# daisy9542/yolo-puncture

Hardware: AMD Instinct MI355X
Metric: images/sec (higher is better)
Workload: dtype bf16

## Files before the change

### include/yolop.h

```cpp
#ifndef YOLOP_H
#define YOLOP_H

#include <stddef.h>
#include <stdint.h>

#ifdef __cplusplus
extern "C" {
#endif

#define YP_OK 0
#define YP_ERR_ARG -1
#define YP_ERR_STATE -2
#define YP_ERR_HIP -3
#define YP_ERR_WEIGHT -4

#define YP_BF16 0
#define YP_F32 1

#define YP_TASK_DETECT 0
#define YP_TASK_SEGMENT 1

#define YP_NM 32
#define YP_MAX_MASKS 480
#define YP_MAX_DET 512
// ... 123 lines not shown
int yp_set_nms(yp_engine* e, float conf, float iou);

int yp_set_attention_form(yp_engine* e, int form);

int yp_set_autotune(yp_engine* e, int enable);

int yp_tuning_export(const yp_engine* e, int32_t* cfg_out, int cap);
int yp_tuning_import(yp_engine* e, int B, int H, int W, const int32_t* cfg, int n);

int yp_debug_force_conv_cfg(int cfg);
int yp_debug_op_cfg(const yp_engine* e, int i, int* cfg);
int yp_debug_last_store_form(void);
int yp_debug_max_workgroups(int n);
int yp_debug_conv_families(int* base, int* num_cfgs, int cap);
int yp_debug_ablation(int v);
int yp_debug_head_clocks(uint64_t* out8);
int yp_debug_attention(const void* qkv_dev, void* o_dev, int dtype, int B, int N, int nh, int kd, int hd, int q_stride, int q_coff, int o_stride,
                       int o_coff, int wgs, int* kernel_out, void* stream);
int yp_debug_attention_form(const void* qkv_dev, void* o_dev, int dtype, int B, int N, int nh, int kd, int hd, int q_stride, int q_coff, int o_stride,
                            int o_coff, int wgs, int form, int* kernel_out, void* stream);
int yp_debug_conv_s2(const void* x_dev, const void* w_dev, const float* bias_dev, const void* res_dev, void* y_dev, int out_f32, int B, int H,
                     int W, int Cin, int Cout, int silu, int cfg, int lds_weights, int64_t* lds_out, char* kernel_out, int kernel_cap,
                     void* stream);
int yp_debug_topk_anchors(const uint32_t* const mk_dev[3], int B, const int hw[3][2], int k, int32_t* sel_out_dev, uint32_t* thr_out_dev, void* stream);
int yp_debug_head_branch_clocks(uint64_t* out8);
int yp_debug_head_winners(yp_engine* e, int32_t* sel_host, float* box_host, float* coeff_host);
int yp_debug_contour_clocks(uint64_t* out12);
int yp_debug_pwsp_clocks(uint64_t* out32);

int yp_tuning_source(const yp_engine* e);

int yp_debug_host_selftest(yp_engine* e);
int yp_debug_graph_info(const yp_engine* e, int64_t* out6);
int yp_debug_head_positions(yp_engine* e, int64_t* out6);
int yp_debug_marker(void* stream);

int yp_set_graph(yp_engine* e, int enable);

#ifdef __cplusplus
}
#endif
#endif
```

### yolo-puncture_amd/csrc/common.h

```cpp
#pragma once
#include <hip/hip_runtime.h>
#include <stdint.h>
#include <atomic>
#include <cstdlib>
#include <string>
#include <vector>

namespace yp {

enum DType { DT_BF16 = 0, DT_F32 = 1 };
enum Act { ACT_NONE = 0, ACT_SILU = 1, ACT_RELU = 2 };

enum OpKind {
    OP_STEM = 0,
    OP_CONV = 1,
    OP_DWCONV = 2,
    OP_POOL5 = 3,
    OP_UPSAMPLE = 4,
    OP_ATTN = 5,
    OP_HEAD = 6,
    OP_CONVT = 7,
    OP_AMAX = 9,
    OP_POOL3 = 8,
};
// ... 253 lines not shown
void conv_dma_force_cfg(int cfg);
int conv_dma_forced_cfg();
void conv_set_debug_ablation(int v);
int conv_debug_ablation();
bool tile_balance_enabled(int family);

struct ConvFamily {
    int base, num_cfgs;
    bool (*valid)(const ConvParams& p, int c);
    std::string (*symbol)(const ConvParams& p, int c);
    hipError_t (*launch)(const ConvParams& p, int c, hipStream_t st);
    bool two_source;
    const char* tune_env;
    bool opt_in;
};
inline const char* res_f32_args(const ConvParams& p) { return p.out_f32 ? ",false,true" : p.res ? ",true,false" : ",false,false"; }
extern const ConvFamily conv_dma_family, conv_halo_family, conv_halo_p_family, conv_dma_p_family, conv_dma_lc_family, conv_halo_s2_family,
    conv_tile1_family, conv_wreg_family, conv_pxd_family, conv_ks_family, conv_wres_family, conv_wrs_family;
constexpr int kNumConvFamilies = 12;
extern const ConvFamily* const kConvFamilies[kNumConvFamilies];
int conv_halo_s2_pw_cfg(const ConvParams& p);
size_t conv_halo_s2_lds_bytes(const ConvParams& p, int c);
int conv_halo_s2_lds_weights(int on);
hipError_t launch_dwconv(const DwParams& p, int dtype, hipStream_t st);
std::string dwconv_kernel_name(const DwParams& p, int dtype);
hipError_t launch_stem(const StemParams& p, int dtype, hipStream_t st);
std::string stem_kernel_name(const StemParams& p, int dtype);
hipError_t launch_pool5(const PoolParams& p, int dtype, hipStream_t st);
hipError_t launch_sppf_pool3(const PoolParams& p, int dtype, hipStream_t st);
bool sppf_pool3_fits(const PoolParams& p, int dtype);
bool dwconv_mfma_valid(const DwParams& p, int dtype);
hipError_t launch_dwconv_mfma(const DwParams& p, hipStream_t st);
const char* dwconv_mfma_kernel_name(const DwParams& p);
hipError_t launch_upsample(const UpParams& p, int dtype, hipStream_t st);
enum AttnForm { ATTN_FORM_AUTO = 0, ATTN_FORM_STREAM = 1, ATTN_FORM_STREAM_WIDE = 3 };
inline bool attn_form_valid(int form) { return form == ATTN_FORM_AUTO || form == ATTN_FORM_STREAM || form == ATTN_FORM_STREAM_WIDE; }
constexpr int ATTN_RESIDENT_TOKENS = 400;
hipError_t launch_attention(const AttnParams& p, int dtype, hipStream_t st, int wgs = 0, int* kernel_out = nullptr, int form = ATTN_FORM_AUTO);
bool attention_fits(const AttnParams& p, int dtype, int* max_tokens, int form = ATTN_FORM_AUTO);
bool attention_takes_stream(const AttnParams& p, int dtype, int form);
bool attention_takes_stream_wide(const AttnParams& p, int dtype, int form);
bool attention_stream_scope(const AttnParams& p, int dtype);
void attention_stream_split(int B, int N, int nh, int wgs, int* nsplit_out, int* gpw_out);
hipError_t launch_attention_stream(const AttnParams& p, hipStream_t st, int wgs);
bool attention_stream_wide_scope(const AttnParams& p, int dtype);
hipError_t launch_attention_stream_wide(const AttnParams& p, hipStream_t st, int wgs);
// ... 118 lines not shown
```

### yolo-puncture_amd/csrc/conv_wres.hip

```cpp
#include "common.h"

namespace yp {

constexpr int WR_NW = 8;
constexpr int WR_MAXNF = 8;

template <int N, int FM, int NFW> __device__ __forceinline__ void wr_wait_lgkm(bf16x8 (&xs)[FM], bf16x8 (&ws)[NFW]) {
    static_assert(N >= 0 && N < 16, "lgkmcnt range");
    asm volatile("s_waitcnt lgkmcnt(%0)" : : "n"(N) : "memory");
#pragma unroll
    for (int f = 0; f < FM; ++f) asm volatile("" : "+v"(xs[f]));
#pragma unroll
    for (int i = 0; i < NFW; ++i) asm volatile("" : "+v"(ws[i]));
}

template <int TP, int WGN> constexpr bool wres_paired() { return (TP / (16 * (WR_NW / WGN))) * (WR_MAXNF / WGN) >= 8; }

template <int TP, int WGN, bool HAS_RES, bool CLK>
__device__ __forceinline__ void conv_wres_body(const ConvParams p, const int NB, const int nblk, const int G, const int TPe) {
    constexpr int WGM = WR_NW / WGN;
    constexpr int FM = TP / (16 * WGM);
    constexpr int NFW = WR_MAXNF / WGN;
    static_assert(FM >= 1 && FM * 16 * WGM == TP, "pixel tile");
    extern __shared__ __attribute__((aligned(1024))) unsigned char smem[];
    const int K = p.Cin, KA = p.x2_C, KB = K - KA;
    const int RBW = K * 2, RBA = KA * 2, RBB = KB * 2;
    const int mA = (KA % 128) == 0 ? 15 : 7, mB = (KB % 128) == 0 ? 15 : 7, mW = ((K % 128) == 0 && (KA % 128) == 0) ? 15 : 7;
    const int nfb = (NB + 15) >> 4;
    const int nfw = nfb / WGN;
    unsigned char* const Ws = smem;
    const size_t xtile = (size_t)TP * RBW;
    unsigned char* const Xs = smem + (size_t)nfb * 16 * RBW;
    const int tid = threadIdx.x, lane = tid & 63;
    const int wave = __builtin_amdgcn_readfirstlane(tid >> 6);
    const int wm = wave % WGM, wn = wave / WGM;
    const int fr = lane & 15, fc = lane >> 4;
    const bool wide = wres_paired<TP, WGN>() && p.wide != 0;
    const int ntiles = (p.M + TPe - 1) / TPe;
    const int HoWo = p.Ho * p.Wo;
    unsigned long long clk[5] = {0, 0, 0, 0, 0}, last = CLK ? __builtin_amdgcn_s_memtime() : 0ull;
#define WRES_STAMP(i) if constexpr (CLK) { const unsigned long long now = __builtin_amdgcn_s_memtime(); clk[i] += now - last; last = now; }

    const int xcd = blockIdx.x & 7, slot = blockIdx.x >> 3;
    const int nb = slot % nblk, g = (slot / nblk) * 8 + xcd;
    const int Gt = G / nblk;
    const int n0 = nb * NB;

    const __amdgpu_buffer_rsrc_t xrs = __builtin_amdgcn_make_buffer_rsrc((void*)p.x, 0, (int)p.x_bytes, 0x00020000);
    const __amdgpu_buffer_rsrc_t x2rs = __builtin_amdgcn_make_buffer_rsrc((void*)(KA > 0 ? p.x2 : p.x), 0, (int)(KA > 0 ? p.x2_bytes : p.x_bytes), 0x00020000);
    const __amdgpu_buffer_rsrc_t wrs = __builtin_amdgcn_make_buffer_rsrc((void*)p.w, 0, (int)p.w_bytes, 0x00020000);
    const __amdgpu_buffer_rsrc_t yrs = __builtin_amdgcn_make_buffer_rsrc((void*)p.y, 0, (int)p.y_bytes, 0x00020000);

    auto issue_tile = [&](int tile, unsigned char* dst) {
        const long row0 = (long)tile * TPe;
        if (KA > 0) {
// ... 6 lines not shown
                unsigned voff = kBufferOOB;
                if (m < p.M && r < TPe) {
                    const int mi = (int)m;
                    const int b = mi / HoWo, q = mi - b * HoWo;
                    const int ho = q / p.Wo, wo = q - ho * p.Wo;
                    voff = (unsigned)((((b * p.x2_H + (ho >> 1)) * p.x2_W + (wo >> 1)) * p.x2_stride + p.x2_coff + c * 8) * 2);
                }
                __builtin_amdgcn_raw_ptr_buffer_load_lds(x2rs, (lds_void*)(dst + ii * 1024), 16, voff, 0, 0, 0);
            }
        }
        {
            unsigned char* const d2 = dst + (size_t)TP * RBA;
            const int cpr = RBB >> 4, pieces = (TP * cpr) >> 6;
            for (int ii = wave; ii < pieces; ii += WR_NW) {
                const int s = ii * 64 + lane;
                const int r = s / cpr, pc = s - r * cpr;
                const int c = pc ^ (r & mB);
                const long m = row0 + r;
                const unsigned voff = (m < p.M && r < TPe) ? (unsigned)((m * p.x_stride + p.x_coff + KA + c * 8) * 2) : kBufferOOB;
                __builtin_amdgcn_raw_ptr_buffer_load_lds(xrs, (lds_void*)(d2 + ii * 1024), 16, voff, 0, 0, 0);
            }
        }
    };
    {
        const int cpr = RBW >> 4, pieces = (nfb * 16 * cpr) >> 6;
        for (int ii = wave; ii < pieces; ii += WR_NW) {
            const int s = ii * 64 + lane;
            const int r = s / cpr, pc = s - r * cpr;
            const int c = pc ^ (r & mW);
            const unsigned voff = (unsigned)(((n0 + weight_row_channel(r, wide)) * p.Kpad + c * 8) * 2);
            __builtin_amdgcn_raw_ptr_buffer_load_lds(wrs, (lds_void*)(Ws + ii * 1024), 16, voff, 0, 0, 0);
        }
    }
    int tile = g;
    if (tile < ntiles) issue_tile(tile, Xs);

    float bias[NFW][4];
#pragma unroll
    for (int i = 0; i < NFW; ++i)
#pragma unroll
        for (int r = 0; r < 4; ++r) {
            const int co = wres_paired<TP, WGN>() ? n0 + wn * nfw * 16 + acc_channel(i, fc, wide) + r : n0 + (wn * nfw + i) * 16 + fc * 4 + r;
            bias[i][r] = (i < nfw && co < p.Cout) ? p.bias[co] : 0.f;
        }
    wait_vmcnt<0>();
#pragma unroll
    for (int i = 0; i < NFW; ++i)
#pragma unroll
        for (int r = 0; r < 4; ++r) asm volatile("" : "+v"(bias[i][r]));

    WRES_STAMP(0)
    for (int it = 0; tile < ntiles; tile += Gt, ++it) {
        if (it == 0) wait_vmcnt<0>();
        else if (wide) wait_vmcnt<FM * NFW / 2>();
        else wait_vmcnt<FM * NFW>();
// ... 26 lines not shown
                for (int i = 0; i < NFW; ++i) asm volatile("ds_read_b128 %0, %1" : "=v"(wd[i]) : "v"(wrow[i] + offw));
            };
            auto mma = [&](bf16x8 (&xd)[FM], bf16x8 (&wd)[NFW]) {
#pragma unroll
                for (int i = 0; i < NFW; ++i)
#pragma unroll
                    for (int f = 0; f < FM; ++f) acc[i][f] = __builtin_amdgcn_mfma_f32_16x16x32_bf16(wd[i], xd[f], acc[i][f], 0, 0, 0);
            };
            bf16x8 xa[FM], wa[NFW], xb[FM], wb[NFW];
            rd(xa, wa, 0);
            for (int ks = 0; ks < nks; ks += 2) {
                rd(xb, wb, ks + 1);
                wr_wait_lgkm<FM + NFW>(xa, wa);
                mma(xa, wa);
                if (ks + 2 < nks) {
                    rd(xa, wa, ks + 2);
                    wr_wait_lgkm<FM + NFW>(xb, wb);
                } else {
                    wr_wait_lgkm<0>(xb, wb);
                }
                mma(xb, wb);
            }
        };
        if (KA > 0) run_segment(XA, RBA, 0, KA >> 5, mA);
        run_segment(XB, RBB, KA >> 3, KB >> 5, mB);
        WRES_STAMP(3)
#pragma unroll
        for (int f = 0; f < FM; ++f) {
            const int ri = (wm * FM + f) * 16 + fr;
            const long m = (long)tile * TPe + ri;
            if (wide) {
#pragma unroll
                for (int j = 0; j < NFW / 2; ++j) {
                    const int co = n0 + wn * nfw * 16 + acc_channel(2 * j, fc, true);
                    const bool ok = 2 * j < nfw && ri < TPe && m < p.M && co < p.Cout;
                    float v[2][4];
#pragma unroll
                    for (int h = 0; h < 2; ++h) {
#pragma unroll
                        for (int q = 0; q < 4; ++q) v[h][q] = acc[2 * j + h][f][q];
                        if (p.act == ACT_SILU && 2 * j < nfw) silu4_packed(v[h]);
                    }
                    if (HAS_RES) {
                        uint2 rr[2];
                        load_res_bf16x8((const __bf16*)p.res + m * p.res_stride + p.res_coff + co, ok, rr[0], rr[1]);
                        add_res_bf16x4(v[0], rr[0]);
                        add_res_bf16x4(v[1], rr[1]);
                    }
// ... 9 lines not shown
                if (p.act == ACT_SILU && i < nfw) silu4_packed(v);
                if (HAS_RES && ok) {
                    const uint2 rr = *(const uint2*)((const __bf16*)p.res + m * p.res_stride + p.res_coff + co);
                    v[0] += __uint_as_float(rr.x << 16); v[1] += __uint_as_float(rr.x & 0xffff0000u);
                    v[2] += __uint_as_float(rr.y << 16); v[3] += __uint_as_float(rr.y & 0xffff0000u);
                }
                __attribute__((aligned(8))) __bf16 o[4] = {(__bf16)v[0], (__bf16)v[1], (__bf16)v[2], (__bf16)v[3]};
                const unsigned off = ok ? (unsigned)((m * p.y_stride + p.y_coff + co) * 2) : kBufferOOB;
                __builtin_amdgcn_raw_buffer_store_b64(*(const __attribute__((ext_vector_type(2))) unsigned*)o, yrs, off, 0, 0);
            }
        }
        WRES_STAMP(4)
    }
    wait_vmcnt<0>();
    if constexpr (CLK) {
        if (lane == 0)
            for (int i = 0; i < 5; ++i) p.clk[((size_t)blockIdx.x * WR_NW + wave) * 5 + i] = clk[i];
    }
#undef WRES_STAMP
}

template <int TP, int WGN, bool HAS_RES>
__global__ __launch_bounds__(WR_NW * 64) void conv_wres_kernel(const ConvParams p, const int NB, const int nblk, const int G, const int TPe) {
    conv_wres_body<TP, WGN, HAS_RES, false>(p, NB, nblk, G, TPe);
}
template <int TP, int WGN>
__global__ __launch_bounds__(WR_NW * 64) void conv_wres_clk_kernel(const ConvParams p, const int NB, const int nblk, const int G, const int TPe) {
    conv_wres_body<TP, WGN, false, true>(p, NB, nblk, G, TPe);
}

struct WresCfg { int TP, WGN; const char* name; };
static const WresCfg kWres[] = {
    {64, 2, "conv_wres_kernel<64,2"},
    {128, 2, "conv_wres_kernel<128,2"},
    {32, 4, "conv_wres_kernel<32,4"},
};
constexpr int kNumWres = (int)(sizeof(kWres) / sizeof(kWres[0]));

static std::string conv_wres_symbol(const ConvParams& p, int c) { return std::string(kWres[c].name) + (p.res ? ",true>" : ",false>"); }

static void wres_blocks(const ConvParams& p, const WresCfg& k, int& NB, int& nblk) {
    nblk = (p.Cout + 127) / 128;
    const int q = 16 * k.WGN;
    NB = ((p.Cout + nblk - 1) / nblk + q - 1) / q * q;
}
static size_t wres_lds(const ConvParams& p, const WresCfg& k) {
    int NB, nblk;
    wres_blocks(p, k, NB, nblk);
    return (size_t)NB * p.Cin * 2 + (size_t)2 * k.TP * p.Cin * 2;
}

static bool conv_wres_cfg_valid(const ConvParams& p, int c) {
    if (c < 0 || c >= kNumWres) return false;
    const WresCfg& k = kWres[c];
    if (p.ks != 1 || p.stride != 1 || p.up != 1 || p.w2 || p.out_f32 || p.pool_in || p.up_bilinear) return false;
    if (p.act != ACT_SILU && p.act != ACT_NONE) return false;
    if (p.Cin < 64 || (p.Cin % 64) != 0 || p.Kpad != p.Cin || p.Cin > 1024) return false;
    if (p.x2_C > 0 && ((p.x2_C % 64) != 0 || p.x2_C >= p.Cin || (p.x2_stride & 7) || (p.x2_coff & 7) || p.x2_bytes >= (1ull << 31))) return false;
    if ((p.x_stride & 7) || (p.x_coff & 7)) return false;
    if ((p.Cout & 3) || (p.y_stride & 3) || (p.y_coff & 3) || (p.res && ((p.res_stride & 3) || (p.res_coff & 3)))) return false;
    if (p.x_bytes >= (1ull << 31) || p.w_bytes >= (1ull << 31) || p.y_bytes >= (1ull << 31) || p.M <= 0 || p.Ho <= 0 || p.Wo <= 0) return false;
    if ((((size_t)k.TP * (p.Cin - p.x2_C) * 2) & 1023) || (((size_t)k.TP * p.x2_C * 2) & 1023)) return false;
    return wres_lds(p, k) <= 156 * 1024;
}

template <int TP, int WGN, bool HAS_RES>
static hipError_t launch_wres_t(const ConvParams& p_in, const WresCfg& k, hipStream_t st) {
    int NB, nblk;
    wres_blocks(p_in, k, NB, nblk);
    const ConvParams p = with_store_form(p_in, wres_paired<TP, WGN>() ? NB / (16 * WGN) : 1);
    const size_t sh = wres_lds(p, k);
    auto kern = conv_wres_kernel<TP, WGN, HAS_RES>;
    static size_t granted = 0;
    if (hipError_t e = allow_dynamic_lds((const void*)kern, sh, granted)) return e;
    const int ntiles = (p.M + TP - 1) / TP;
    const int gmax = sh <= 78 * 1024 ? 512 : 256;
    int lanes8 = gmax / (8 * nblk);
    if (lanes8 < 1) lanes8 = 1;
    while (lanes8 > 1 && (lanes8 - 1) * 8 >= ntiles) --lanes8;
    if (const int cap = debug_max_workgroups()) while (lanes8 > 1 && lanes8 * 8 * nblk > cap) --lanes8;
    const int G = lanes8 * 8 * nblk;
    const long lanes = (long)lanes8 * 8;
    const int rounds = (int)((p.M + lanes * TP - 1) / (lanes * TP));
    const int TPe = tile_balance_enabled(2) ? (int)((p.M + lanes * rounds - 1) / (lanes * rounds)) : TP;
    if constexpr (TP == 128 && WGN == 2 && !HAS_RES) {
        static const bool clocks = env_on("YOLOP_WRES_CLOCKS");
        if (clocks) {
            auto kc = conv_wres_clk_kernel<TP, WGN>;
            static size_t granted_c = 0;
            if (hipError_t e = allow_dynamic_lds((const void*)kc, sh, granted_c)) return e;
            ConvParams q = p;
            const size_t n = (size_t)G * WR_NW * 5;
            if (hipMalloc((void**)&q.clk, n * 8) != hipSuccess) return hipErrorOutOfMemory;
            hipLaunchKernelGGL(kc, dim3((unsigned)G), dim3(WR_NW * 64), sh, st, q, NB, nblk, G, TPe);
            (void)hipStreamSynchronize(st);
            std::vector<unsigned long long> h(n);
            (void)hipMemcpy(h.data(), q.clk, n * 8, hipMemcpyDeviceToHost);
            (void)hipFree(q.clk);
            double s5[5] = {0, 0, 0, 0, 0};
            for (size_t w = 0; w < n / 5; ++w)
                for (int i = 0; i < 5; ++i) s5[i] += (double)h[w * 5 + i];
            fprintf(stderr, "[wres clocks] %s G=%d tiles=%d  %s stores  per-wave mean cycles: prologue %.0f  wait+barrier %.0f  issue %.0f  k loop %.0f  epilogue %.0f\n",
                    k.name, G, (p.M + TPe - 1) / TPe, p.wide ? "16-byte" : "8-byte", s5[0] / (n / 5), s5[1] / (n / 5), s5[2] / (n / 5), s5[3] / (n / 5), s5[4] / (n / 5));
            return hipGetLastError();
        }
    }
    hipLaunchKernelGGL(kern, dim3((unsigned)G), dim3(WR_NW * 64), sh, st, p, NB, nblk, G, TPe);
    return hipGetLastError();
}

static hipError_t launch_conv_wres(const ConvParams& p, int c, hipStream_t st) {
    if (!conv_wres_cfg_valid(p, c)) return hipErrorInvalidValue;
    const WresCfg& k = kWres[c];
    const bool r = p.res != nullptr;
    switch (c) {
        case 0: return r ? launch_wres_t<64, 2, true>(p, k, st) : launch_wres_t<64, 2, false>(p, k, st);
        case 1: return r ? launch_wres_t<128, 2, true>(p, k, st) : launch_wres_t<128, 2, false>(p, k, st);
        default: return r ? launch_wres_t<32, 4, true>(p, k, st) : launch_wres_t<32, 4, false>(p, k, st);
    }
}

#if !defined(__HIP_DEVICE_COMPILE__)
const ConvFamily conv_wres_family = {1100, kNumWres, conv_wres_cfg_valid, conv_wres_symbol, launch_conv_wres, true, "YOLOP_NO_WRES", false};
#endif

}
```

### yolo-puncture_amd/csrc/engine.hip

```cpp
#include "../../include/yolop.h"
#include "common.h"
#include <algorithm>
#include <array>
#include <chrono>

#include <cmath>
#include <cstdarg>
#include <cstdio>
#include <cstring>
#include <cstdlib>
#include <dlfcn.h>
#include <fcntl.h>
#include <fstream>
#include <map>
#include <sstream>
#include <memory>

using namespace yp;

static thread_local char g_err[512] = "";
static int fail(int code, const char* fmt, ...) {
    va_list ap;
    va_start(ap, fmt);
    vsnprintf(g_err, sizeof(g_err), fmt, ap);
// ... 2389 lines not shown
    p.M = B * p.Ho * p.Wo;
    p.ks = 3; p.stride = 2; p.pad = 1; p.up = 1;
    p.act = silu ? ACT_SILU : ACT_NONE; p.out_f32 = out_f32 ? 1 : 0;
    p.x_bytes = (size_t)B * H * W * Cin * 2; p.w_bytes = (size_t)Cout * 9 * Cin * 2; p.y_bytes = (size_t)p.M * Cout * esz;
    p.cfg = -1;
    const int before = conv_halo_s2_lds_weights(lds_weights ? 1 : 0);
    const bool ok = f.valid(p, cfg - f.base);
    hipError_t err = hipSuccess;
    if (lds_out) *lds_out = (int64_t)conv_halo_s2_lds_bytes(p, cfg - f.base);
    if (ok && kernel_out && kernel_cap > 0) std::snprintf(kernel_out, (size_t)kernel_cap, "%s", f.symbol(p, cfg - f.base).c_str());
    if (ok && !host_only) {
        hipStream_t st = (hipStream_t)stream;
        err = f.launch(p, cfg - f.base, st);
        if (err == hipSuccess) err = hipStreamSynchronize(st);
    }
    conv_halo_s2_lds_weights(before);
    if (!ok)
        return fail(YP_ERR_ARG, "yp_debug_conv_s2: configuration %d does not admit B %d, H %d, W %d, Cin %d, Cout %d%s%s%s", cfg, B, H, W, Cin, Cout,
                    res_dev ? ", residual" : "", out_f32 ? ", fp32 output" : "", lds_weights ? ", weights in LDS" : "");
    if (err != hipSuccess) return fail(YP_ERR_HIP, "yp_debug_conv_s2: %s", hipGetErrorString(err));
    return YP_OK;
}

int yp_tuning_source(const yp_engine* e) {
    if (!e) return YP_ERR_ARG;
    return e->tune_source;
}

int yp_debug_graph_info(const yp_engine* e, int64_t* out6) {
    if (!e || !out6) return fail(YP_ERR_ARG, "yp_debug_graph_info: null argument");
    out6[0] = e->n_captures; out6[1] = e->g_nodes; out6[2] = e->g_edges; out6[3] = e->g_edges_expected;
    out6[4] = (int64_t)e->lanes_used.size() + 1; out6[5] = e->gexec ? 1 : 0;
    return YP_OK;
}

int yp_debug_head_positions(yp_engine* e, int64_t* out6) {
    if (!e || !out6) return fail(YP_ERR_ARG, "yp_debug_head_positions: null argument");
    for (int i = 0; i < 6; ++i) out6[i] = 0;
    if (!e->allocated) return fail(YP_ERR_STATE, "no forward has run yet");
    const Op* h = nullptr;
    for (const Op& o : e->ops) if (o.kind == OP_HEAD) h = &o;
    if (!h || !(h->sparse_box || h->sparse_cf) || !e->sp_ws) return 0;
    HIPCHK(hipSetDevice(e->device));
    HIPCHK(hipDeviceSynchronize());
    const SparseWs ws = sparse_ws_layout(*e);
    const char* base = (const char*)e->sp_ws;
// ... 366 lines not shown
```

### yolo-puncture_amd/engine.py

```python
from __future__ import annotations

import ctypes as C
import os
from typing import Dict, List, Optional, Tuple

import numpy as np
import torch

from .weights import fold_state

_LIB: Optional[C.CDLL] = None
_HERE = os.path.dirname(os.path.abspath(__file__))
LIB_PATH = os.environ.get("YOLOP_LIB") or os.path.join(_HERE, "libyolop.so")

YP_BF16, YP_F32 = 0, 1
TASK_DETECT, TASK_SEGMENT = 0, 1
OP_KINDS = {0: "stem", 1: "conv", 2: "dwconv", 3: "pool5", 4: "upsample", 5: "attn", 6: "head", 7: "convT", 8: "pool3", 9: "amax"}
FORMS = ("plain", "dwpw", "dwpw_tail", "s2pw", "frontend", "c2f", "scdown", "pwsp", "cls_out")


class ModelDesc(C.Structure):
    _fields_ = [("variant", C.c_int), ("nc", C.c_int), ("task", C.c_int), ("dtype", C.c_int), ("max_det", C.c_int), ("family", C.c_int)]


# ... 23 lines not shown
    lib.yp_masks.argtypes = [vp, C.c_int, vp, vp, C.c_int, C.c_int, C.c_int, C.c_int, vp, vp, vp, C.c_int, C.c_int, vp]
    lib.yp_id_mask_resized.argtypes = [vp, C.c_int, vp, vp] + [C.c_int] * 5 + [vp, vp, C.c_int, C.c_int, vp]
    lib.yp_id_mask_resized.restype = C.c_int
    lib.yp_mask_contours.argtypes = [vp, C.c_int, C.c_int, C.c_int, C.c_int, vp, vp, vp, vp]
    lib.yp_mask_contours.restype = C.c_int
    lib.yp_mask_contours_scaled.argtypes = [vp, C.c_int, C.c_int, C.c_int, C.c_int, C.c_int, vp, vp, vp, C.c_int, vp, C.c_int, C.c_int, vp]
    lib.yp_mask_contours_scaled.restype = C.c_int
    lib.yp_mask_contours_large_workspace.argtypes = [C.c_int, C.c_int, C.c_int]
    lib.yp_mask_contours_large_workspace.restype = C.c_size_t
    lib.yp_mask_contours_large.argtypes = [vp, C.c_int, C.c_int, C.c_int, C.c_int, C.c_int, vp, vp, vp, C.c_int, vp, C.c_int, C.c_int, C.c_int, vp,
                                           C.c_size_t, vp]
    lib.yp_mask_contours_large.restype = C.c_int
    lib.yp_plan.argtypes = [vp, C.c_int, C.c_int, C.c_int]
    lib.yp_max_batch.argtypes = [vp, C.c_int, C.c_int]
    lib.yp_max_batch.restype = C.c_int
    lib.yp_debug_topk_anchors.argtypes = [C.POINTER(vp), C.c_int, C.POINTER(C.c_int), C.c_int, vp, vp, vp]
    lib.yp_debug_topk_anchors.restype = C.c_int
    lib.yp_debug_attention.argtypes = [vp, vp] + [C.c_int] * 11 + [ip, vp]
    lib.yp_debug_attention.restype = C.c_int
    lib.yp_debug_attention_form.argtypes = [vp, vp] + [C.c_int] * 12 + [ip, vp]
    lib.yp_debug_attention_form.restype = C.c_int
    lib.yp_debug_conv_s2.argtypes = [vp, vp, vp, vp, vp] + [C.c_int] * 9 + [C.POINTER(C.c_int64), C.c_char_p, C.c_int, vp]
    lib.yp_debug_conv_s2.restype = C.c_int
    lib.yp_set_attention_form.argtypes = [vp, C.c_int]
    lib.yp_set_attention_form.restype = C.c_int
    lib.yp_op_info.argtypes = [vp, C.c_int, C.c_char_p, C.c_int, ip, C.POINTER(C.c_double), C.POINTER(C.c_double)]
    lib.yp_op_output.argtypes = [vp, C.c_int, ip, ip, ip]
    lib.yp_op_kernel.argtypes = [vp, C.c_int, C.c_char_p, C.c_int]
    lib.yp_op_fusion.argtypes = [vp, C.c_int, ip, ip]
    lib.yp_op_fusion.restype = C.c_int
    lib.yp_debug_op_form.argtypes = [vp, C.c_int, ip, ip, C.c_int]
    lib.yp_debug_op_form.restype = C.c_int
    lib.yp_run_op.argtypes = [vp, C.c_int, vp, vp, vp, vp, vp]
    lib.yp_tensor_write.argtypes = [vp, C.c_int, C.c_int, C.c_int, vp]
    lib.yp_tensor_count.argtypes = [vp]
    lib.yp_tensor_info.argtypes = [vp, C.c_int, C.c_char_p, C.c_int, ip, ip]
    lib.yp_tensor_read.argtypes = [vp, C.c_int, vp]
    lib.yp_profile.argtypes = [vp, vp, C.c_int, C.c_int, C.c_int, vp, vp, vp, vp, C.c_int, vp]
    lib.yp_set_graph.argtypes = [vp, C.c_int]
    lib.yp_set_autotune.argtypes = [vp, C.c_int]
    lib.yp_set_nms.argtypes = [vp, C.c_float, C.c_float]
    lib.yp_set_nms.restype = C.c_int
    lib.yp_debug_host_selftest.argtypes = [vp]
    lib.yp_debug_host_selftest.restype = C.c_int
    lib.yp_tuning_source.argtypes = [vp]
    lib.yp_tuning_source.restype = C.c_int
# ... 24 lines not shown
    lib.yp_masks_frames.argtypes = [vp, vp, C.c_int, vp, C.c_long, vp, C.c_int, C.c_int, vp, vp]
    lib.yp_masks_frames.restype = C.c_int
    lib.yp_masks_frames_input.argtypes = [vp, vp, C.c_int, vp, C.c_long, vp, C.c_int, C.c_int, vp, vp]
    lib.yp_masks_frames_input.restype = C.c_int
    lib.yp_comm_unique_id.argtypes = [vp]
    lib.yp_comm_create.argtypes = [vp, C.c_int, C.c_int, C.c_int, C.POINTER(vp)]
    lib.yp_allgather.argtypes = [vp, vp, vp, C.c_size_t, vp]
    lib.yp_comm_destroy.argtypes = [vp]
    for fn in ("yp_comm_unique_id", "yp_comm_create", "yp_allgather", "yp_comm_destroy"):
        getattr(lib, fn).restype = C.c_int
    for fn in ("yp_create", "yp_destroy", "yp_weight_count", "yp_weight_info", "yp_set_weight", "yp_finalize",
               "yp_forward", "yp_proto", "yp_masks", "yp_plan", "yp_op_info", "yp_op_output", "yp_op_input", "yp_tensor_count",
               "yp_tensor_info", "yp_tensor_read", "yp_profile", "yp_set_graph", "yp_run_op", "yp_tensor_write",
               "yp_op_kernel", "yp_set_autotune", "yp_debug_force_conv_cfg", "yp_debug_ablation"):
        getattr(lib, fn).restype = C.c_int
    if path is None:
        _LIB = lib
    return lib


EXPORTS = ["yp_last_error", "yp_create", "yp_destroy", "yp_weight_count", "yp_weight_info", "yp_set_weight",
           "yp_finalize", "yp_forward", "yp_proto", "yp_masks", "yp_id_mask_resized", "yp_plan", "yp_op_info", "yp_op_output", "yp_op_input", "yp_op_fusion",
           "yp_tensor_count", "yp_tensor_info", "yp_tensor_read", "yp_profile", "yp_set_graph", "yp_run_op",
           "yp_tensor_write", "yp_op_kernel", "yp_set_autotune", "yp_tuning_export", "yp_tuning_import", "yp_set_nms", "yp_debug_force_conv_cfg", "yp_debug_op_cfg", "yp_debug_op_form", "yp_debug_last_store_form", "yp_debug_max_workgroups", "yp_debug_conv_families", "yp_debug_ablation", "yp_debug_head_clocks", "yp_debug_head_branch_clocks", "yp_debug_head_winners", "yp_debug_contour_clocks", "yp_debug_pwsp_clocks", "yp_debug_host_selftest", "yp_debug_graph_info", "yp_tuning_source", "yp_debug_head_positions", "yp_debug_marker", "yp_max_batch", "yp_debug_topk_anchors", "yp_debug_attention", "yp_debug_attention_form", "yp_debug_conv_s2", "yp_set_attention_form", "yp_letterbox", "yp_letterbox_batch", "yp_masks_frames", "yp_masks_frames_input", "yp_mask_contours",
           "yp_mask_contours_scaled", "yp_mask_contours_large_workspace", "yp_mask_contours_large", "yp_comm_unique_id", "yp_comm_create", "yp_allgather", "yp_comm_destroy",
           "yp_u2net_create", "yp_u2net_destroy", "yp_u2net_weight_count", "yp_u2net_weight_info", "yp_u2net_set_weight", "yp_u2net_finalize",
           "yp_u2net_forward", "yp_u2net_forward_crops", "yp_u2net_set_graph", "yp_u2net_tensor_count", "yp_u2net_tensor_info", "yp_u2net_tensor_read",
           "yp_u2net_op_count", "yp_u2net_op_info",
           "yp_cls_create", "yp_cls_destroy", "yp_cls_weight_count", "yp_cls_weight_info", "yp_cls_set_weight", "yp_cls_finalize",
           "yp_cls_forward", "yp_cls_set_graph", "yp_cls_tensor_count", "yp_cls_tensor_info", "yp_cls_tensor_read"]


MAX_ANCHORS = 294912
ATTENTION_FORMS = {"auto": 0, "stream": 1, "stream_wide": 3}


def _attention_form(form) -> int:
    if form not in ATTENTION_FORMS:
        raise ValueError(f"attention form {form!r}: one of {sorted(ATTENTION_FORMS)}")
    return ATTENTION_FORMS[form]


def topk_anchors(mk: List[torch.Tensor], hw, k: int) -> Tuple[torch.Tensor, torch.Tensor]:
    lib = load_library()
    if len(mk) != 3 or len(hw) != 3:
        raise ValueError("three levels")
    B = int(mk[0].shape[0])
# ... 39 lines not shown
    Cout = int(w.shape[0])
    if tuple(w.shape) != (Cout, 3, 3, Cin) or tuple(bias.shape) != (Cout,) or not (x.is_cuda and w.is_cuda and bias.is_cuda):
        raise ValueError("w must be [Cout, 3, 3, Cin] and bias [Cout], all on the device")
    if not (x.is_contiguous() and w.is_contiguous() and bias.is_contiguous()):
        raise ValueError("contiguous tensors")
    if res is not None and (res.dtype != torch.bfloat16 or tuple(res.shape) != (B, H // 2, W // 2, Cout) or not res.is_contiguous() or res.device != x.device):
        raise ValueError("res must be a contiguous bf16 [B, H/2, W/2, Cout] on x's device")
    y = torch.zeros((B, H // 2, W // 2, Cout), dtype=torch.float32 if out_f32 else torch.bfloat16, device=x.device)
    rc = lib.yp_debug_conv_s2(C.c_void_p(x.data_ptr()), C.c_void_p(w.data_ptr()), C.c_void_p(bias.data_ptr()),
                              C.c_void_p(res.data_ptr()) if res is not None else None, C.c_void_p(y.data_ptr()), int(bool(out_f32)), B, H, W, Cin, Cout,
                              int(bool(silu)), int(cfg), int(bool(lds_weights)), None, None, 0, C.c_void_p(_stream_ptr(x.device)))
    if rc < 0:
        raise YolopError(lib.yp_last_error().decode())
    return y


def conv_s2_admits(cfg: int, B: int, H: int, W: int, Cin: int, Cout: int, res: bool = False, out_f32: bool = False,
                   lds_weights: bool = False) -> Tuple[bool, int, str]:
    lib = load_library()
    lds = C.c_int64(0)
    name = C.create_string_buffer(160)
    rc = lib.yp_debug_conv_s2(None, None, None, C.c_void_p(1) if res else None, None, int(bool(out_f32)), int(B), int(H), int(W), int(Cin), int(Cout),
                              1, int(cfg), int(bool(lds_weights)), C.byref(lds), name, 160, None)
    return rc >= 0, int(lds.value), name.value.decode()


def conv_families() -> List[Tuple[int, int]]:
    lib = load_library()
    n = lib.yp_debug_conv_families(None, None, 0)
    base, num = (C.c_int * n)(), (C.c_int * n)()
    lib.yp_debug_conv_families(base, num, n)
    return list(zip(base, num))


def _stream_ptr(device: torch.device) -> int:
    return int(torch.cuda.current_stream(device).cuda_stream)


def letterbox_device(src: torch.Tensor, geo: dict, out: Optional[torch.Tensor] = None, pad_value: int = 114) -> torch.Tensor:
    if not (src.is_cuda and src.dtype == torch.uint8 and src.dim() == 3 and src.shape[2] == 3 and src.is_contiguous()):
        raise ValueError("letterbox_device needs a contiguous uint8 CUDA tensor [H,W,3]")
    oh, ow = int(geo["out_h"]), int(geo["out_w"])
    if out is None:
        out = torch.empty((oh, ow, 3), dtype=torch.uint8, device=src.device)
    if not (out.is_cuda and out.dtype == torch.uint8 and tuple(out.shape) == (oh, ow, 3) and out.is_contiguous()):
        raise ValueError(f"letterbox_device: output must be a contiguous uint8 CUDA tensor [{oh},{ow},3]")
# ... 404 lines not shown
```

Before: 22930.

## Hold conv weights in registers for small-Cin weights-resident 1x1 convs

Adds a register-weights variant of the weights-resident pointwise conv kernel. For single-source inputs with Cin of 128/192/256 (depending on config), each wave loads its weight fragments from LDS into VGPRs once in the prologue. The weight LDS region is then dropped, so LDS holds only the double-buffered pixel tiles and the K loop issues only activation ds_reads. This cuts LDS traffic and footprint at the cost of up to 144 extra VGPRs, which may lower occupancy; the 512-workgroup grid is now allowed only when the register budget is small. An env switch restores LDS weights, and a debug entry point plus Python wrapper are added.

Measured after the change: 23130 (median of 6 runs). No clear change (+0.9%).

```diff
diff --git a/include/yolop.h b/include/yolop.h
--- a/include/yolop.h
+++ b/include/yolop.h
@@ -169,6 +169,9 @@
 int yp_debug_conv_s2(const void* x_dev, const void* w_dev, const float* bias_dev, const void* res_dev, void* y_dev, int out_f32, int B, int H,
                      int W, int Cin, int Cout, int silu, int cfg, int lds_weights, int64_t* lds_out, char* kernel_out, int kernel_cap,
                      void* stream);
+int yp_debug_conv_wres(const void* x_dev, const void* w_dev, const float* bias_dev, const void* res_dev, void* y_dev, int B, int H, int W, int Cin,
+                       int Cout, int x_stride, int x_coff, int y_stride, int y_coff, int silu, int cfg, int lds_weights, int64_t* lds_out,
+                       char* kernel_out, int kernel_cap, void* stream);
 int yp_debug_topk_anchors(const uint32_t* const mk_dev[3], int B, const int hw[3][2], int k, int32_t* sel_out_dev, uint32_t* thr_out_dev, void* stream);
 int yp_debug_head_branch_clocks(uint64_t* out8);
 int yp_debug_head_winners(yp_engine* e, int32_t* sel_host, float* box_host, float* coeff_host);
diff --git a/yolo-puncture_amd/csrc/common.h b/yolo-puncture_amd/csrc/common.h
--- a/yolo-puncture_amd/csrc/common.h
+++ b/yolo-puncture_amd/csrc/common.h
@@ -299,6 +299,8 @@
 int conv_halo_s2_pw_cfg(const ConvParams& p);
 size_t conv_halo_s2_lds_bytes(const ConvParams& p, int c);
 int conv_halo_s2_lds_weights(int on);
+size_t conv_wres_lds_bytes(const ConvParams& p, int c);
+int conv_wres_lds_weights(int on);
 hipError_t launch_dwconv(const DwParams& p, int dtype, hipStream_t st);
 std::string dwconv_kernel_name(const DwParams& p, int dtype);
 hipError_t launch_stem(const StemParams& p, int dtype, hipStream_t st);
diff --git a/yolo-puncture_amd/csrc/conv_wres.hip b/yolo-puncture_amd/csrc/conv_wres.hip
--- a/yolo-puncture_amd/csrc/conv_wres.hip
+++ b/yolo-puncture_amd/csrc/conv_wres.hip
@@ -4,6 +4,8 @@
 
 constexpr int WR_NW = 8;
 constexpr int WR_MAXNF = 8;
+constexpr int kWresWregMaxVgprs = 144;
+constexpr int kWresLdsMax = 156 * 1024;
 
 template <int N, int FM, int NFW> __device__ __forceinline__ void wr_wait_lgkm(bf16x8 (&xs)[FM], bf16x8 (&ws)[NFW]) {
     static_assert(N >= 0 && N < 16, "lgkmcnt range");
@@ -13,24 +15,32 @@
 #pragma unroll
     for (int i = 0; i < NFW; ++i) asm volatile("" : "+v"(ws[i]));
 }
+template <int N, int FM> __device__ __forceinline__ void wr_wait_lgkm_x(bf16x8 (&xs)[FM]) {
+    static_assert(N >= 0 && N < 16, "lgkmcnt range");
+    asm volatile("s_waitcnt lgkmcnt(%0)" : : "n"(N) : "memory");
+#pragma unroll
+    for (int f = 0; f < FM; ++f) asm volatile("" : "+v"(xs[f]));
+}
 
 template <int TP, int WGN> constexpr bool wres_paired() { return (TP / (16 * (WR_NW / WGN))) * (WR_MAXNF / WGN) >= 8; }
 
-template <int TP, int WGN, bool HAS_RES, bool CLK>
+template <int TP, int WGN, bool HAS_RES, bool CLK, int NKS>
 __device__ __forceinline__ void conv_wres_body(const ConvParams p, const int NB, const int nblk, const int G, const int TPe) {
     constexpr int WGM = WR_NW / WGN;
     constexpr int FM = TP / (16 * WGM);
     constexpr int NFW = WR_MAXNF / WGN;
     static_assert(FM >= 1 && FM * 16 * WGM == TP, "pixel tile");
+    constexpr bool WREG = NKS > 0;
+    static_assert(!WREG || ((NKS & 1) == 0 && NFW * NKS * 4 <= kWresWregMaxVgprs), "register-weights instance");
     extern __shared__ __attribute__((aligned(1024))) unsigned char smem[];
-    const int K = p.Cin, KA = p.x2_C, KB = K - KA;
+    const int K = WREG ? NKS * 32 : p.Cin, KA = WREG ? 0 : p.x2_C, KB = K - KA;
     const int RBW = K * 2, RBA = KA * 2, RBB = KB * 2;
     const int mA = (KA % 128) == 0 ? 15 : 7, mB = (KB % 128) == 0 ? 15 : 7, mW = ((K % 128) == 0 && (KA % 128) == 0) ? 15 : 7;
     const int nfb = (NB + 15) >> 4;
     const int nfw = nfb / WGN;
     unsigned char* const Ws = smem;
     const size_t xtile = (size_t)TP * RBW;
-    unsigned char* const Xs = smem + (size_t)nfb * 16 * RBW;
+    unsigned char* const Xs = WREG ? smem : smem + (size_t)nfb * 16 * RBW;
     const int tid = threadIdx.x, lane = tid & 63;
     const int wave = __builtin_amdgcn_readfirstlane(tid >> 6);
     const int wm = wave % WGM, wn = wave / WGM;
@@ -83,7 +93,8 @@
             }
         }
     };
-    {
+    bf16x8 wr[WREG ? NFW : 1][WREG ? NKS : 1];
+    if constexpr (!WREG) {
         const int cpr = RBW >> 4, pieces = (nfb * 16 * cpr) >> 6;
         for (int ii = wave; ii < pieces; ii += WR_NW) {
             const int s = ii * 64 + lane;
@@ -92,6 +103,37 @@
             const unsigned voff = (unsigned)(((n0 + weight_row_channel(r, wide)) * p.Kpad + c * 8) * 2);
             __builtin_amdgcn_raw_ptr_buffer_load_lds(wrs, (lds_void*)(Ws + ii * 1024), 16, voff, 0, 0, 0);
         }
+    } else {
+        constexpr int CPR = NKS * 4;
+        constexpr int PF = 2 * TP / 16;
+        for (int f0 = 0; f0 < nfb; f0 += PF) {
+            const int nf = min(PF, nfb - f0);
+            const int pieces = (nf * 16 * CPR) >> 6;
+            for (int ii = wave; ii < pieces; ii += WR_NW) {
+                const int s = ii * 64 + lane;
+                const int r = s / CPR, pc = s - r * CPR;
+                const int c = pc ^ (r & mW);
+                const unsigned voff = (unsigned)(((n0 + weight_row_channel(f0 * 16 + r, wide)) * p.Kpad + c * 8) * 2);
+                __builtin_amdgcn_raw_ptr_buffer_load_lds(wrs, (lds_void*)(smem + ii * 1024), 16, voff, 0, 0, 0);
+            }
+            wait_vmcnt<0>();
+            __builtin_amdgcn_s_barrier();
+#pragma unroll
+            for (int i = 0; i < NFW; ++i) {
+                const int fi = wn * nfw + min(i, nfw - 1) - f0;
+                if (fi >= 0 && fi < nf) {
+#pragma unroll
+                    for (int ks = 0; ks < NKS; ++ks)
+                        wr[i][ks] = *(const bf16x8*)(smem + (size_t)(fi * 16 + fr) * RBW + (((ks * 4 + fc) ^ (fr & mW)) << 4));
+                }
+            }
+            __builtin_amdgcn_s_waitcnt(0xc07f);
+            __builtin_amdgcn_s_barrier();
+        }
+#pragma unroll
+        for (int i = 0; i < NFW; ++i)
+#pragma unroll
+            for (int ks = 0; ks < NKS; ++ks) asm volatile("" : "+v"(wr[i][ks]));
     }
     int tile = g;
     if (tile < ntiles) issue_tile(tile, Xs);
@@ -164,8 +206,45 @@
                 mma(xb, wb);
             }
         };
-        if (KA > 0) run_segment(XA, RBA, 0, KA >> 5, mA);
-        run_segment(XB, RBB, KA >> 3, KB >> 5, mB);
+        if constexpr (WREG) {
+            auto run_wreg = [&]() {
+                unsigned xrow[FM];
+                const unsigned xl = (unsigned)(size_t)(const __attribute__((address_space(3))) unsigned char*)XB;
+#pragma unroll
+                for (int f = 0; f < FM; ++f) xrow[f] = xl + (unsigned)(((wm * FM + f) * 16 + fr) * RBB);
+                const unsigned swx = (unsigned)(fr & mB);
+                auto rd = [&](bf16x8 (&xd)[FM], int ks) {
+                    const unsigned offx = (((unsigned)(ks * 4 + fc)) ^ swx) << 4;
+#pragma unroll
+                    for (int f = 0; f < FM; ++f) asm volatile("ds_read_b128 %0, %1" : "=v"(xd[f]) : "v"(xrow[f] + offx));
+                };
+                auto mma = [&](bf16x8 (&xd)[FM], int ks) {
+#pragma unroll
+                    for (int i = 0; i < NFW; ++i)
+#pragma unroll
+                        for (int f = 0; f < FM; ++f) acc[i][f] = __builtin_amdgcn_mfma_f32_16x16x32_bf16(wr[i][ks], xd[f], acc[i][f], 0, 0, 0);
+                };
+                bf16x8 xa[FM], xb[FM];
+                rd(xa, 0);
+#pragma unroll
+                for (int ks = 0; ks < NKS; ks += 2) {
+                    rd(xb, ks + 1);
+                    wr_wait_lgkm_x<FM>(xa);
+                    mma(xa, ks);
+                    if (ks + 2 < NKS) {
+                        rd(xa, ks + 2);
+                        wr_wait_lgkm_x<FM>(xb);
+                    } else {
+                        wr_wait_lgkm_x<0>(xb);
+                    }
+                    mma(xb, ks + 1);
+                }
+            };
+            run_wreg();
+        } else {
+            if (KA > 0) run_segment(XA, RBA, 0, KA >> 5, mA);
+            run_segment(XB, RBB, KA >> 3, KB >> 5, mB);
+        }
         WRES_STAMP(3)
 #pragma unroll
         for (int f = 0; f < FM; ++f) {
@@ -221,11 +300,21 @@
 
 template <int TP, int WGN, bool HAS_RES>
 __global__ __launch_bounds__(WR_NW * 64) void conv_wres_kernel(const ConvParams p, const int NB, const int nblk, const int G, const int TPe) {
-    conv_wres_body<TP, WGN, HAS_RES, false>(p, NB, nblk, G, TPe);
+    conv_wres_body<TP, WGN, HAS_RES, false, 0>(p, NB, nblk, G, TPe);
 }
 template <int TP, int WGN>
 __global__ __launch_bounds__(WR_NW * 64) void conv_wres_clk_kernel(const ConvParams p, const int NB, const int nblk, const int G, const int TPe) {
-    conv_wres_body<TP, WGN, false, true>(p, NB, nblk, G, TPe);
+    conv_wres_body<TP, WGN, false, true, 0>(p, NB, nblk, G, TPe);
+}
+template <int TP, int WGN, bool HAS_RES, int NKS>
+__global__ __launch_bounds__(WR_NW * 64) void conv_wres_kernel(const ConvParams p, const int NB, const int nblk, const int G, const int TPe) {
+    static_assert(NKS > 0, "the fourth argument is a register-weights instance's substep count");
+    conv_wres_body<TP, WGN, HAS_RES, false, NKS>(p, NB, nblk, G, TPe);
+}
+template <int TP, int WGN, int NKS>
+__global__ __launch_bounds__(WR_NW * 64) void conv_wres_clk_kernel(const ConvParams p, const int NB, const int nblk, const int G, const int TPe) {
+    static_assert(NKS > 0, "the third argument is a register-weights instance's substep count");
+    conv_wres_body<TP, WGN, false, true, NKS>(p, NB, nblk, G, TPe);
 }
 
 struct WresCfg { int TP, WGN; const char* name; };
@@ -236,18 +325,40 @@
 };
 constexpr int kNumWres = (int)(sizeof(kWres) / sizeof(kWres[0]));
 
-static std::string conv_wres_symbol(const ConvParams& p, int c) { return std::string(kWres[c].name) + (p.res ? ",true>" : ",false>"); }
+static std::atomic<int>& wres_lds_weights_ref() {
+    static std::atomic<int> v{env_on("YOLOP_WRES_LDS_WEIGHTS") ? 1 : 0};
+    return v;
+}
+int conv_wres_lds_weights(int on) { return on < 0 ? wres_lds_weights_ref().load() : wres_lds_weights_ref().exchange(on ? 1 : 0); }
+
+static int wres_wreg_nks(const ConvParams& p, int c) {
+    if (p.x2_C > 0 || (p.Cin % 64) != 0 || wres_lds_weights_ref().load()) return 0;
+    const int nks = p.Cin / 32;
+    if ((WR_MAXNF / kWres[c].WGN) * nks * 4 > kWresWregMaxVgprs) return 0;
+    switch (c) {
+        case 0: return (nks == 6 || nks == 8) ? nks : 0;
+        case 1: return nks == 4 ? nks : 0;
+        default: return nks == 8 ? nks : 0;
+    }
+}
+static std::string conv_wres_symbol(const ConvParams& p, int c) {
+    const int nks = wres_wreg_nks(p, c);
+    return std::string(kWres[c].name) + (p.res ? ",true" : ",false") + (nks ? "," + std::to_string(nks) : std::string()) + ">";
+}
 
 static void wres_blocks(const ConvParams& p, const WresCfg& k, int& NB, int& nblk) {
     nblk = (p.Cout + 127) / 128;
     const int q = 16 * k.WGN;
     NB = ((p.Cout + nblk - 1) / nblk + q - 1) / q * q;
 }
-static size_t wres_lds(const ConvParams& p, const WresCfg& k) {
+static size_t wres_lds(const ConvParams& p, const WresCfg& k, int nks) {
+    const size_t tile = (size_t)k.TP * p.Cin * 2;
+    if (nks > 0) return 2 * tile;
     int NB, nblk;
     wres_blocks(p, k, NB, nblk);
-    return (size_t)NB * p.Cin * 2 + (size_t)2 * k.TP * p.Cin * 2;
-}
+    return (size_t)NB * p.Cin * 2 + 2 * tile;
+}
+size_t conv_wres_lds_bytes(const ConvParams& p, int c) { return (c >= 0 && c < kNumWres) ? wres_lds(p, kWres[c], wres_wreg_nks(p, c)) : 0; }
 
 static bool conv_wres_cfg_valid(const ConvParams& p, int c) {
     if (c < 0 || c >= kNumWres) return false;
@@ -260,20 +371,25 @@
     if ((p.Cout & 3) || (p.y_stride & 3) || (p.y_coff & 3) || (p.res && ((p.res_stride & 3) || (p.res_coff & 3)))) return false;
     if (p.x_bytes >= (1ull << 31) || p.w_bytes >= (1ull << 31) || p.y_bytes >= (1ull << 31) || p.M <= 0 || p.Ho <= 0 || p.Wo <= 0) return false;
     if ((((size_t)k.TP * (p.Cin - p.x2_C) * 2) & 1023) || (((size_t)k.TP * p.x2_C * 2) & 1023)) return false;
-    return wres_lds(p, k) <= 156 * 1024;
-}
-
-template <int TP, int WGN, bool HAS_RES>
+    return wres_lds(p, k, wres_wreg_nks(p, c)) <= (size_t)kWresLdsMax;
+}
+
+template <int TP, int WGN, int... NKS> constexpr bool wres_two_per_cu() {
+    return sizeof...(NKS) == 0 || ((WR_MAXNF / WGN) * (0 + ... + NKS) * 4 <= 64 && TP == 16 * (WR_NW / WGN));
+}
+
+template <int TP, int WGN, bool HAS_RES, int... NKS>
 static hipError_t launch_wres_t(const ConvParams& p_in, const WresCfg& k, hipStream_t st) {
+    constexpr int nks = (0 + ... + NKS);
     int NB, nblk;
     wres_blocks(p_in, k, NB, nblk);
     const ConvParams p = with_store_form(p_in, wres_paired<TP, WGN>() ? NB / (16 * WGN) : 1);
-    const size_t sh = wres_lds(p, k);
-    auto kern = conv_wres_kernel<TP, WGN, HAS_RES>;
+    const size_t sh = wres_lds(p, k, nks);
+    auto kern = conv_wres_kernel<TP, WGN, HAS_RES, NKS...>;
     static size_t granted = 0;
     if (hipError_t e = allow_dynamic_lds((const void*)kern, sh, granted)) return e;
     const int ntiles = (p.M + TP - 1) / TP;
-    const int gmax = sh <= 78 * 1024 ? 512 : 256;
+    const int gmax = (sh <= 78 * 1024 && wres_two_per_cu<TP, WGN, NKS...>()) ? 512 : 256;
     int lanes8 = gmax / (8 * nblk);
     if (lanes8 < 1) lanes8 = 1;
     while (lanes8 > 1 && (lanes8 - 1) * 8 >= ntiles) --lanes8;
@@ -282,10 +398,10 @@
     const long lanes = (long)lanes8 * 8;
     const int rounds = (int)((p.M + lanes * TP - 1) / (lanes * TP));
     const int TPe = tile_balance_enabled(2) ? (int)((p.M + lanes * rounds - 1) / (lanes * rounds)) : TP;
-    if constexpr (TP == 128 && WGN == 2 && !HAS_RES) {
+    if constexpr (!HAS_RES) {
         static const bool clocks = env_on("YOLOP_WRES_CLOCKS");
         if (clocks) {
-            auto kc = conv_wres_clk_kernel<TP, WGN>;
+            auto kc = conv_wres_clk_kernel<TP, WGN, NKS...>;
             static size_t granted_c = 0;
             if (hipError_t e = allow_dynamic_lds((const void*)kc, sh, granted_c)) return e;
             ConvParams q = p;
@@ -299,23 +415,32 @@
             double s5[5] = {0, 0, 0, 0, 0};
             for (size_t w = 0; w < n / 5; ++w)
                 for (int i = 0; i < 5; ++i) s5[i] += (double)h[w * 5 + i];
-            fprintf(stderr, "[wres clocks] %s G=%d tiles=%d  %s stores  per-wave mean cycles: prologue %.0f  wait+barrier %.0f  issue %.0f  k loop %.0f  epilogue %.0f\n",
-                    k.name, G, (p.M + TPe - 1) / TPe, p.wide ? "16-byte" : "8-byte", s5[0] / (n / 5), s5[1] / (n / 5), s5[2] / (n / 5), s5[3] / (n / 5), s5[4] / (n / 5));
+            fprintf(stderr, "[wres clocks] %s,false%s> G=%d tiles=%d  %s stores  per-wave mean cycles: prologue %.0f  wait+barrier %.0f  issue %.0f  k loop %.0f  epilogue %.0f\n",
+                    k.name, nks ? ("," + std::to_string(nks)).c_str() : "", G, (p.M + TPe - 1) / TPe, p.wide ? "16-byte" : "8-byte", s5[0] / (n / 5), s5[1] / (n / 5), s5[2] / (n / 5), s5[3] / (n / 5), s5[4] / (n / 5));
             return hipGetLastError();
         }
     }
     hipLaunchKernelGGL(kern, dim3((unsigned)G), dim3(WR_NW * 64), sh, st, p, NB, nblk, G, TPe);
     return hipGetLastError();
+}
+
+template <int TP, int WGN, int... NKS>
+static hipError_t launch_wres_r(const ConvParams& p, const WresCfg& k, hipStream_t st) {
+    return p.res ? launch_wres_t<TP, WGN, true, NKS...>(p, k, st) : launch_wres_t<TP, WGN, false, NKS...>(p, k, st);
 }
 
 static hipError_t launch_conv_wres(const ConvParams& p, int c, hipStream_t st) {
     if (!conv_wres_cfg_valid(p, c)) return hipErrorInvalidValue;
     const WresCfg& k = kWres[c];
-    const bool r = p.res != nullptr;
-    switch (c) {
-        case 0: return r ? launch_wres_t<64, 2, true>(p, k, st) : launch_wres_t<64, 2, false>(p, k, st);
-        case 1: return r ? launch_wres_t<128, 2, true>(p, k, st) : launch_wres_t<128, 2, false>(p, k, st);
-        default: return r ? launch_wres_t<32, 4, true>(p, k, st) : launch_wres_t<32, 4, false>(p, k, st);
+    switch (c * 100 + wres_wreg_nks(p, c)) {
+        case 0: return launch_wres_r<64, 2>(p, k, st);
+        case 6: return launch_wres_r<64, 2, 6>(p, k, st);
+        case 8: return launch_wres_r<64, 2, 8>(p, k, st);
+        case 100: return launch_wres_r<128, 2>(p, k, st);
+        case 104: return launch_wres_r<128, 2, 4>(p, k, st);
+        case 200: return launch_wres_r<32, 4>(p, k, st);
+        case 208: return launch_wres_r<32, 4, 8>(p, k, st);
+        default: return hipErrorInvalidValue;
     }
 }
 
diff --git a/yolo-puncture_amd/csrc/engine.hip b/yolo-puncture_amd/csrc/engine.hip
--- a/yolo-puncture_amd/csrc/engine.hip
+++ b/yolo-puncture_amd/csrc/engine.hip
@@ -2435,6 +2435,50 @@
     return YP_OK;
 }
 
+int yp_debug_conv_wres(const void* x_dev, const void* w_dev, const float* bias_dev, const void* res_dev, void* y_dev, int B, int H, int W, int Cin,
+                       int Cout, int x_stride, int x_coff, int y_stride, int y_coff, int silu, int cfg, int lds_weights, int64_t* lds_out,
+                       char* kernel_out, int kernel_cap, void* stream) {
+    if (lds_out) *lds_out = 0;
+    if (kernel_out && kernel_cap > 0) kernel_out[0] = 0;
+    const bool host_only = !x_dev && !w_dev && !bias_dev && !y_dev;
+    if (!host_only && (!x_dev || !w_dev || !bias_dev || !y_dev)) return fail(YP_ERR_ARG, "yp_debug_conv_wres: null argument");
+    if (B < 1 || H < 1 || W < 1 || Cin < 1 || Cout < 1)
+        return fail(YP_ERR_ARG, "yp_debug_conv_wres: non-positive size (B %d, H %d, W %d, Cin %d, Cout %d)", B, H, W, Cin, Cout);
+    if (x_coff < 0 || y_coff < 0 || (int64_t)x_coff + Cin > x_stride || (int64_t)y_coff + Cout > y_stride)
+        return fail(YP_ERR_ARG, "yp_debug_conv_wres: the slices [%d, %d + %d) of x_stride %d / [%d, %d + %d) of y_stride %d do not fit", x_coff, x_coff, Cin,
+                    x_stride, y_coff, y_coff, Cout, y_stride);
+    const ConvFamily& f = conv_wres_family;
+    if (cfg < f.base || cfg >= f.base + f.num_cfgs)
+        return fail(YP_ERR_ARG, "yp_debug_conv_wres: cfg = %d is no id of the weights-resident family [%d, %d)", cfg, f.base, f.base + f.num_cfgs);
+    ConvParams p{};
+    p.x = x_dev; p.x_stride = x_stride; p.x_coff = x_coff; p.H = H; p.W = W; p.Cin = Cin;
+    p.w = w_dev; p.Kpad = Cin; p.bias = bias_dev;
+    p.Ho = H; p.Wo = W; p.Cout = Cout;
+    p.y = y_dev; p.y_stride = y_stride; p.y_coff = y_coff;
+    p.res = res_dev; p.res_stride = Cout; p.res_coff = 0;
+    p.M = B * H * W;
+    p.ks = 1; p.stride = 1; p.pad = 0; p.up = 1;
+    p.act = silu ? ACT_SILU : ACT_NONE; p.wide = 1;
+    p.x_bytes = (size_t)p.M * x_stride * 2; p.w_bytes = (size_t)Cout * Cin * 2; p.y_bytes = (size_t)p.M * y_stride * 2;
+    p.cfg = -1;
+    const int before = conv_wres_lds_weights(lds_weights ? 1 : 0);
+    const bool ok = f.valid(p, cfg - f.base);
+    hipError_t err = hipSuccess;
+    if (lds_out) *lds_out = (int64_t)conv_wres_lds_bytes(p, cfg - f.base);
+    if (ok && kernel_out && kernel_cap > 0) std::snprintf(kernel_out, (size_t)kernel_cap, "%s", f.symbol(p, cfg - f.base).c_str());
+    if (ok && !host_only) {
+        hipStream_t st = (hipStream_t)stream;
+        err = f.launch(p, cfg - f.base, st);
+        if (err == hipSuccess) err = hipStreamSynchronize(st);
+    }
+    conv_wres_lds_weights(before);
+    if (!ok)
+        return fail(YP_ERR_ARG, "yp_debug_conv_wres: configuration %d does not admit B %d, H %d, W %d, Cin %d, Cout %d, x_stride %d, x_coff %d, y_stride %d, y_coff %d%s%s",
+                    cfg, B, H, W, Cin, Cout, x_stride, x_coff, y_stride, y_coff, res_dev ? ", residual" : "", lds_weights ? ", weights in LDS" : "");
+    if (err != hipSuccess) return fail(YP_ERR_HIP, "yp_debug_conv_wres: %s", hipGetErrorString(err));
+    return YP_OK;
+}
+
 int yp_tuning_source(const yp_engine* e) {
     if (!e) return YP_ERR_ARG;
     return e->tune_source;
diff --git a/yolo-puncture_amd/engine.py b/yolo-puncture_amd/engine.py
--- a/yolo-puncture_amd/engine.py
+++ b/yolo-puncture_amd/engine.py
@@ -69,6 +69,8 @@
     lib.yp_debug_attention_form.restype = C.c_int
     lib.yp_debug_conv_s2.argtypes = [vp, vp, vp, vp, vp] + [C.c_int] * 9 + [C.POINTER(C.c_int64), C.c_char_p, C.c_int, vp]
     lib.yp_debug_conv_s2.restype = C.c_int
+    lib.yp_debug_conv_wres.argtypes = [vp, vp, vp, vp, vp] + [C.c_int] * 12 + [C.POINTER(C.c_int64), C.c_char_p, C.c_int, vp]
+    lib.yp_debug_conv_wres.restype = C.c_int
     lib.yp_set_attention_form.argtypes = [vp, C.c_int]
     lib.yp_set_attention_form.restype = C.c_int
     lib.yp_op_info.argtypes = [vp, C.c_int, C.c_char_p, C.c_int, ip, C.POINTER(C.c_double), C.POINTER(C.c_double)]
@@ -139,7 +141,7 @@
 EXPORTS = ["yp_last_error", "yp_create", "yp_destroy", "yp_weight_count", "yp_weight_info", "yp_set_weight",
            "yp_finalize", "yp_forward", "yp_proto", "yp_masks", "yp_id_mask_resized", "yp_plan", "yp_op_info", "yp_op_output", "yp_op_input", "yp_op_fusion",
            "yp_tensor_count", "yp_tensor_info", "yp_tensor_read", "yp_profile", "yp_set_graph", "yp_run_op",
-           "yp_tensor_write", "yp_op_kernel", "yp_set_autotune", "yp_tuning_export", "yp_tuning_import", "yp_set_nms", "yp_debug_force_conv_cfg", "yp_debug_op_cfg", "yp_debug_op_form", "yp_debug_last_store_form", "yp_debug_max_workgroups", "yp_debug_conv_families", "yp_debug_ablation", "yp_debug_head_clocks", "yp_debug_head_branch_clocks", "yp_debug_head_winners", "yp_debug_contour_clocks", "yp_debug_pwsp_clocks", "yp_debug_host_selftest", "yp_debug_graph_info", "yp_tuning_source", "yp_debug_head_positions", "yp_debug_marker", "yp_max_batch", "yp_debug_topk_anchors", "yp_debug_attention", "yp_debug_attention_form", "yp_debug_conv_s2", "yp_set_attention_form", "yp_letterbox", "yp_letterbox_batch", "yp_masks_frames", "yp_masks_frames_input", "yp_mask_contours",
+           "yp_tensor_write", "yp_op_kernel", "yp_set_autotune", "yp_tuning_export", "yp_tuning_import", "yp_set_nms", "yp_debug_force_conv_cfg", "yp_debug_op_cfg", "yp_debug_op_form", "yp_debug_last_store_form", "yp_debug_max_workgroups", "yp_debug_conv_families", "yp_debug_ablation", "yp_debug_head_clocks", "yp_debug_head_branch_clocks", "yp_debug_head_winners", "yp_debug_contour_clocks", "yp_debug_pwsp_clocks", "yp_debug_host_selftest", "yp_debug_graph_info", "yp_tuning_source", "yp_debug_head_positions", "yp_debug_marker", "yp_max_batch", "yp_debug_topk_anchors", "yp_debug_attention", "yp_debug_attention_form", "yp_debug_conv_s2", "yp_debug_conv_wres", "yp_set_attention_form", "yp_letterbox", "yp_letterbox_batch", "yp_masks_frames", "yp_masks_frames_input", "yp_mask_contours",
            "yp_mask_contours_scaled", "yp_mask_contours_large_workspace", "yp_mask_contours_large", "yp_comm_unique_id", "yp_comm_create", "yp_allgather", "yp_comm_destroy",
            "yp_u2net_create", "yp_u2net_destroy", "yp_u2net_weight_count", "yp_u2net_weight_info", "yp_u2net_set_weight", "yp_u2net_finalize",
            "yp_u2net_forward", "yp_u2net_forward_crops", "yp_u2net_set_graph", "yp_u2net_tensor_count", "yp_u2net_tensor_info", "yp_u2net_tensor_read",
@@ -225,6 +227,43 @@
     name = C.create_string_buffer(160)
     rc = lib.yp_debug_conv_s2(None, None, None, C.c_void_p(1) if res else None, None, int(bool(out_f32)), int(B), int(H), int(W), int(Cin), int(Cout),
                               1, int(cfg), int(bool(lds_weights)), C.byref(lds), name, 160, None)
+    return rc >= 0, int(lds.value), name.value.decode()
+
+
+def conv_wres(x: torch.Tensor, w: torch.Tensor, bias: torch.Tensor, cfg: int, res: Optional[torch.Tensor] = None, silu: bool = True,
+              lds_weights: bool = False, x_coff: int = 0, out: Optional[torch.Tensor] = None, y_coff: int = 0) -> torch.Tensor:
+    lib = load_library()
+    if x.dim() != 4 or w.dim() != 2 or x.dtype != torch.bfloat16 or w.dtype != torch.bfloat16 or bias.dtype != torch.float32:
+        raise ValueError("x: bf16 [B, H, W, x_stride], w: bf16 [Cout, Cin], bias: float32 [Cout]")
+    B, H, W, x_stride = (int(v) for v in x.shape)
+    Cout, Cin = (int(v) for v in w.shape)
+    if tuple(bias.shape) != (Cout,) or not (x.is_cuda and w.is_cuda and bias.is_cuda):
+        raise ValueError("bias must be [Cout], all tensors on the device")
+    if not (x.is_contiguous() and w.is_contiguous() and bias.is_contiguous()):
+        raise ValueError("contiguous tensors")
+    if res is not None and (res.dtype != torch.bfloat16 or tuple(res.shape) != (B, H, W, Cout) or not res.is_contiguous() or res.device != x.device):
+        raise ValueError("res must be a contiguous bf16 [B, H, W, Cout] on x's device")
+    if out is None:
+        out = torch.zeros((B, H, W, Cout), dtype=torch.bfloat16, device=x.device)
+    if out.dim() != 4 or out.dtype != torch.bfloat16 or tuple(out.shape[:3]) != (B, H, W) or not out.is_contiguous() or out.device != x.device:
+        raise ValueError("out must be a contiguous bf16 [B, H, W, y_stride] on x's device")
+    rc = lib.yp_debug_conv_wres(C.c_void_p(x.data_ptr()), C.c_void_p(w.data_ptr()), C.c_void_p(bias.data_ptr()),
+                                C.c_void_p(res.data_ptr()) if res is not None else None, C.c_void_p(out.data_ptr()), B, H, W, Cin, Cout, x_stride,
+                                int(x_coff), int(out.shape[3]), int(y_coff), int(bool(silu)), int(cfg), int(bool(lds_weights)), None, None, 0,
+                                C.c_void_p(_stream_ptr(x.device)))
+    if rc < 0:
+        raise YolopError(lib.yp_last_error().decode())
+    return out
+
+
+def conv_wres_admits(cfg: int, B: int, H: int, W: int, Cin: int, Cout: int, res: bool = False, lds_weights: bool = False,
+                     x_stride: Optional[int] = None, x_coff: int = 0, y_stride: Optional[int] = None, y_coff: int = 0) -> Tuple[bool, int, str]:
+    lib = load_library()
+    lds = C.c_int64(0)
+    name = C.create_string_buffer(160)
+    rc = lib.yp_debug_conv_wres(None, None, None, C.c_void_p(1) if res else None, None, int(B), int(H), int(W), int(Cin), int(Cout),
+                                int(Cin if x_stride is None else x_stride), int(x_coff), int(Cout if y_stride is None else y_stride), int(y_coff),
+                                1, int(cfg), int(bool(lds_weights)), C.byref(lds), name, 160, None)
     return rc >= 0, int(lds.value), name.value.decode()
 
 
```
